# isi-vista/VistaOCR

Measured on AMD Instinct MI355X. Metric: line-images/sec (train, batch 32, 30x600 grey), higher is better.
Workload: dtype f32 (the LSTM's large GEMMs as bf16x6 products: fp32 operands split exactly into three bf16 planes, six bf16 MFMAs per fp32 product, fp32 accumulate; VOCR_LSTM_GEMM=f32 restores the f32-MFMA kernels); 1 GPU; configs[1]: 32 synthetic 1x30x600 grey lines per GPU, 20 labels/line, V=96, 3xBiLSTM-512, train() = H2D of the batch + fwd+CTC+bwd+allreduce+clamp+Adam, loss returned as a float; widths=600 .. 600 px, mean 600, conv_dtype=fp32, global_batch=32, parallelism=dp1, ranks_seen=1, backend=none, per_rank_rng=seed 1234 + 1000*rank after an identical init

## Files before the change

### include/vocr.h

```cpp
#ifndef VOCR_H
#define VOCR_H
#include <stddef.h>
#include <stdint.h>

#ifdef __cplusplus
extern "C" {
#endif

#define VOCR_OK          0
#define VOCR_EINVAL     -1
#define VOCR_ELAUNCH    -2
#define VOCR_ENODEVICE  -3
#define VOCR_ECOMM      -4


const char* vocr_last_error(void);
#define VOCR_ABI_VERSION 5
int  vocr_abi_version(void);
int  vocr_profile_range_push(const char* name);
int  vocr_profile_range_pop(void);
int  vocr_device_count(void);

int vocr_conv3x3_pack_weights(const float* w, float* wpack_fwd, float* wpack_dgrad, int cout, int cin, void* stream);
int vocr_conv3x3_fwd(const float* x, const float* wpack, const float* bias, float* y,
// ... 111 lines not shown

size_t vocr_gemm_x6_planes_bytes(int rows, int k);
int vocr_gemm_x6_split(const float* x, const float* x2, int seg, int seg_axis, const float* mask, long ld, int rows, int k, int k_contiguous,
                       void* planes, void* stream);
size_t vocr_gemm_x6_workspace_bytes(int m, int n, int k);
#define VOCR_GEMM_X6_PLAN_INTS 9
int vocr_gemm_x6_plan(int m, int n, int k, int b_rows, int b_row0, int b_row0_2, int has_workspace, int* plan);
int vocr_gemm_x6(const void* a_planes, int a_rows, int a_k, int a_row0, int a_kk0, const void* b_planes, int b_rows, int b_k, int b_row0, int b_kk0,
                 int m, int n, int k, float* c0, float* c1, int csplit, int rsplit, int ldc, const float* bias0, const float* bias1, int relu,
                 void* workspace, void* stream);

int vocr_gemm_x6_two_views(const void* a_planes, int a_rows, int a_k, int a_row0, const void* b_planes, int b_rows, int b_k, int m, int n, int k,
                           int rsplit, int a_kk0, int b_row0, int b_kk0, int a_kk0_2, int b_row0_2, int b_kk0_2, float* c0, float* c1, int ldc,
                           void* workspace, void* stream);

size_t vocr_gemm_h3_planes_bytes(int rows, int k);
int vocr_gemm_h3_split(const float* x, const float* x2, int seg, int seg_axis, const float* mask, long ld, int rows, int k, int k_contiguous,
                       float bound, void* planes, void* stream);
int vocr_gemm_h3(const void* a_planes, int a_rows, int a_k, int a_row0, int a_kk0, const void* b_planes, int b_rows, int b_k, int b_row0, int b_kk0,
                 int m, int n, int k, float* c0, float* c1, int csplit, int rsplit, int ldc, const float* bias0, const float* bias1, int relu,
                 void* workspace, void* stream);
int vocr_gemm_h3_two_views(const void* a_planes, int a_rows, int a_k, int a_row0, const void* b_planes, int b_rows, int b_k, int m, int n, int k,
                           int rsplit, int a_kk0, int b_row0, int b_kk0, int a_kk0_2, int b_row0_2, int b_kk0_2, float* c0, float* c1, int ldc,
                           void* workspace, void* stream);

int vocr_lstm_packed_supported(int b, int h);
int vocr_seq_rowmap(const int32_t* lens, int t, int b, int rows, int32_t* to_packed, int32_t* to_dense, void* stream);
int vocr_gather_rows(const float* src, float* dst, const int32_t* map, long nrows, int n, const float* fill, void* stream);
size_t vocr_gather_rows_fill_grad_workspace_bytes(int n);
int vocr_gather_rows_fill_grad(const float* dout, const int32_t* map, long nrows, int n, float* dfill, void* workspace, void* stream);
// ... 119 lines not shown
```

### vistaocr_amd/_lib.py

```python
import ctypes
import os
from ctypes import c_char_p, c_float, c_int, c_size_t, c_uint32, c_uint64, c_void_p

_HERE = os.path.dirname(os.path.abspath(__file__))
LIB_PATH = os.path.join(_HERE, "csrc", "libvocr.so")

P, I, F, Z, U64, U32 = c_void_p, c_int, c_float, c_size_t, c_uint64, c_uint32

SIGNATURES = {
    "vocr_last_error": (c_char_p, []),
    "vocr_abi_version": (I, []),
    "vocr_device_count": (I, []),
    "vocr_profile_range_push": (I, [c_char_p]),
    "vocr_profile_range_pop": (I, []),
    "vocr_conv3x3_pack_weights": (I, [P, P, P, I, I, P]),
    "vocr_conv3x3_fwd": (I, [P, P, P, P, I, I, I, I, I, P]),
    "vocr_conv3x3_wgrad_workspace_bytes": (Z, [I, I, I, I, I]),
    "vocr_conv3x3_wgrad": (I, [P, P, P, P, I, I, I, I, I, P]),
    "vocr_conv3x3_wino_supported": (I, [I, I]),
    "vocr_conv3x3_wino_pack_floats": (Z, [I, I]),
    "vocr_conv3x3_wino_pack_weights": (I, [P, P, P, I, I, P]),
    "vocr_conv3x3_wino_fwd": (I, [P, P, P, P, I, I, I, I, I, P]),
    "vocr_conv3x3_wino_plan": (I, [I, I, I, I, I]),
    "vocr_conv3x3_wgrad_wino_workspace_bytes": (Z, [I, I, I, I, I]),
# ... 28 lines not shown
    "vocr_bn_relu_fracpool2x2_fwd": (I, [P, P, P, P, P, P, P, P, I, I, I, I, I, I, P]),
    "vocr_fracpool2x2_bwd": (I, [P, P, P, I, I, I, I, I, I, P]),
    "vocr_relu_maxpool2_fwd": (I, [P, P, P, I, I, I, I, P]),
    "vocr_relu_maxpool2_bwd": (I, [P, P, P, P, I, I, I, I, P]),
    "vocr_gemm_workspace_bytes": (Z, [I, I, I, I]),
    "vocr_gemm": (I, [I, I, I, I, I, P, I, P, I, P, I, P, I, I, P, Z, P]),
    "vocr_gemm_plan": (I, [I, I, I, I, I, I, I, I, I, I, I, Z, I, I, I, P]),
    "vocr_gemm_pair_workspace_bytes": (Z, [I, I, I, I]),
    "vocr_gemm_pair": (I, [I, I, I, I, I, I, P, P, I, P, P, I, P, P, I, P, P, I, P, Z, P]),
    "vocr_gemm_x6_planes_bytes": (Z, [I, I]),
    "vocr_gemm_x6_split": (I, [P, P, I, I, P, ctypes.c_long, I, I, I, P, P]),
    "vocr_gemm_x6_workspace_bytes": (Z, [I, I, I]),
    "vocr_gemm_x6_plan": (I, [I, I, I, I, I, I, I, P]),
    "vocr_gemm_x6": (I, [P, I, I, I, I, P, I, I, I, I, I, I, I, P, P, I, I, I, P, P, I, P, P]),
    "vocr_gemm_x6_two_views": (I, [P, I, I, I, P, I, I, I, I, I, I, I, I, I, I, I, I, P, P, I, P, P]),
    "vocr_gemm_h3_two_views": (I, [P, I, I, I, P, I, I, I, I, I, I, I, I, I, I, I, I, P, P, I, P, P]),
    "vocr_gemm_h3_planes_bytes": (Z, [I, I]),
    "vocr_gemm_h3_split": (I, [P, P, I, I, P, ctypes.c_long, I, I, I, ctypes.c_float, P, P]),
    "vocr_gemm_h3": (I, [P, I, I, I, I, P, I, I, I, I, I, I, I, P, P, I, I, I, P, P, I, P, P]),
    "vocr_colsum_workspace_bytes": (Z, [I, I]),
    "vocr_colsum": (I, [P, P, I, I, P, P]),
    "vocr_relu_bwd": (I, [P, P, P, Z, P]),
    "vocr_bchw_to_wbch": (I, [P, P, I, I, I, I, P]),
    "vocr_wbch_to_bchw": (I, [P, P, I, I, I, I, P]),
    "vocr_mul": (I, [P, P, P, Z, P]),
    "vocr_add": (I, [P, P, P, Z, P]),
    "vocr_scale_dev": (I, [P, P, P, Z, P]),
    "vocr_dropout_fwd": (I, [P, P, P, Z, F, U64, P]),
    "vocr_dropout_mask": (I, [P, Z, F, U64, P]),
    "vocr_lstm_workspace_bytes": (Z, [I, I, I]),
# ... 138 lines not shown
```

### vistaocr_amd/csrc/gemm_x6.hip

```cpp
#include "vocr_common.h"

namespace {

typedef __bf16 bf16x8 __attribute__((ext_vector_type(8)));
typedef unsigned u32x4x __attribute__((ext_vector_type(4)));
#define X6_LDS_PTR(p) ((__attribute__((address_space(3))) void*)(p))
#define X6_H(v) __builtin_bit_cast(f16x8, v)

constexpr int X6_BM = 256;
constexpr int X6_LDS = 144 * 1024;

__device__ __forceinline__ void split3(float a, __bf16& b0, __bf16& b1, __bf16& b2) {
    b0 = (__bf16)a;
    if (__builtin_isinf((float)b0) && !__builtin_isinf(a)) b0 = __builtin_bit_cast(__bf16, (unsigned short)(__float_as_uint(a) >> 16));
    const float r1 = a - (float)b0;
    b1 = (__bf16)r1;
    const float r2 = r1 - (float)b1;
    b2 = (__bf16)r2;
}

struct X6Src {
    const float* x;
    const float* x2;
    const float* mask;
// ... 187 lines not shown
    const float* sb;
};

constexpr int X6_PANEL = 4;
__device__ __forceinline__ void x6_tile_of(int t, int mtiles, int ntiles, int& mt, int& nt) {
    const int panel = t / (X6_PANEL * ntiles), within = t - panel * X6_PANEL * ntiles;
    const int rows = min(X6_PANEL, mtiles - panel * X6_PANEL);
    nt = within / rows;
    mt = panel * X6_PANEL + within - nt * rows;
}
__device__ __forceinline__ int x6_xcd_chunked(int i, int n) {
    const int xcd = i & 7, j = i >> 3, c = n >> 3, rr = n & 7;
    return xcd * c + min(xcd, rr) + j;
}

template <int NCT, int NP>
__global__ __launch_bounds__(512) void gemm_x6_kernel(const X6Args g) {
    constexpr int BN = 32 * NCT;
    constexpr int TM = NCT == 4 ? 2 : 4, TN = 2;
    constexpr int NA = 8 * NP;
    constexpr int NFRAG = NA + NP * NCT;
    constexpr int NS = NP == 3 ? (NCT == 4 ? 4 : 3) : (NCT == 4 ? 6 : 4);
    constexpr int STAGE = NFRAG * 1024;
    constexpr int NDMA_MAX = (NFRAG + 7) / 8;
    constexpr int NDMA_LO = NFRAG / 8, NDMA_ODD = NFRAG % 8;
    extern __shared__ __attribute__((aligned(1024))) unsigned char lds[];
    const int tid = threadIdx.x, lane = tid & 63;
    const int wave = __builtin_amdgcn_readfirstlane(tid >> 6);
    const int wm = NCT == 4 ? (wave & 3) : (wave & 1), wn = NCT == 4 ? (wave >> 2) : (wave >> 1);
    const int v = x6_xcd_chunked(blockIdx.x, gridDim.x);
    const int ltile = v % g.ntile_launch, split = v / g.ntile_launch;
    int mt, nt;
    x6_tile_of(g.tile0 + ltile, g.mtiles, g.ntiles, mt, nt);
    const int s_beg = split * g.stages_per_split, s_end = min(g.nkk, s_beg + g.stages_per_split);
    if (s_beg >= s_end) return;

    const long pa = (long)g.RTa * g.KKa * 1024, pb = (long)g.RTb * g.KKb * 1024;
    const bool alt = mt >= g.alt_mt;
    const int a_kk0 = alt ? g.a_kk0_alt : g.a_kk0, b_kk0 = alt ? g.b_kk0_alt : g.b_kk0, b_rt0 = alt ? g.b_rt0_alt : g.b_rt0;
    const __amdgpu_buffer_rsrc_t ra = __builtin_amdgcn_make_buffer_rsrc((void*)g.a, 0, (int)(NP * pa), 0x00020000);
    const __amdgpu_buffer_rsrc_t rb = __builtin_amdgcn_make_buffer_rsrc((void*)g.b, 0, (int)(NP * pb), 0x00020000);
    const int voff = lane * 16;
    auto dma_one = [&](int s, int slot, int i) {
        const int f = wave + 8 * i;
        unsigned char* dst = lds + slot * STAGE + f * 1024;
        const bool live = s < s_end;
#if defined(X6_CUT) && (X6_CUT & 16)
        s = s_beg;
#endif
        if (f < NA) {
            const long off = (f >> 3) * pa + ((long)(g.a_rt0 + 8 * mt + (f & 7)) * g.KKa + a_kk0 + s) * 1024;
            __builtin_amdgcn_raw_ptr_buffer_load_lds(ra, X6_LDS_PTR(dst), 16, live ? voff : -16, live ? (int)off : 0, 0, 0);
        } else {
            const int fb = f - NA;
            const long off = (fb / NCT) * pb + ((long)(b_rt0 + NCT * nt + (fb % NCT)) * g.KKb + b_kk0 + s) * 1024;
            __builtin_amdgcn_raw_ptr_buffer_load_lds(rb, X6_LDS_PTR(dst), 16, live ? voff : -16, live ? (int)off : 0, 0, 0);
        }
    };
    auto dma_nth = [&](int s, int slot, int i) {
        if (8 * i + 7 < NFRAG || wave + 8 * i < NFRAG) dma_one(s, slot, i);
    };

    f32x16 acc[TM][TN];
#pragma unroll
    for (int i = 0; i < TM; ++i)
#pragma unroll
        for (int j = 0; j < TN; ++j)
#pragma unroll
            for (int r = 0; r < 16; ++r) acc[i][j][r] = 0.f;

#pragma unroll
    for (int i = 0; i < NS - 1; ++i)
#pragma unroll
        for (int d = 0; d < NDMA_MAX; ++d) dma_nth(s_beg + i, i, d);
#ifndef X6_CUT
#define X6_CUT 0
#endif
    int slot = 0;
    for (int s = s_beg; s < s_end; ++s) {
        if (!(X6_CUT & 1) && !(X6_CUT & 32)) {
            static_assert((NS - 2) * (NDMA_LO + (NDMA_ODD ? 1 : 0)) < 16, "vmcnt immediate");
            if (NDMA_ODD && wave < NDMA_ODD) __builtin_amdgcn_s_waitcnt(0x0F70 | ((NS - 2) * (NDMA_LO + 1)));
            else __builtin_amdgcn_s_waitcnt(0x0F70 | ((NS - 2) * NDMA_LO));
        }
        if (!(X6_CUT & 8)) __builtin_amdgcn_s_barrier();
        const unsigned char* base = lds + slot * STAGE + lane * 16;
        bf16x8 af[TM][NP], bf[TN][NP];
#pragma unroll
        for (int tn = 0; tn < TN; ++tn)
#pragma unroll
            for (int p = 0; p < NP; ++p) bf[tn][p] = *(const bf16x8*)(base + (NA + p * NCT + TN * wn + tn) * 1024);
#pragma unroll
        for (int tm = 0; tm < TM; ++tm)
#pragma unroll
            for (int p = 0; p < NP; ++p) af[tm][p] = *(const bf16x8*)(base + (p * 8 + TM * wm + tm) * 1024);
        __builtin_amdgcn_sched_barrier(0);
        const int snext = s + NS - 1, slot_next = slot == 0 ? NS - 1 : slot - 1;
        int d = 0;
#pragma unroll
        for (int tm = 0; tm < TM; ++tm)
#pragma unroll
            for (int tn = 0; tn < TN; ++tn) {
                if (!(X6_CUT & 2)) {
                    if constexpr (NP == 3) {
                        acc[tm][tn] = __builtin_amdgcn_mfma_f32_32x32x16_bf16(af[tm][1], bf[tn][1], acc[tm][tn], 0, 0, 0);
                        acc[tm][tn] = __builtin_amdgcn_mfma_f32_32x32x16_bf16(af[tm][0], bf[tn][2], acc[tm][tn], 0, 0, 0);
                        acc[tm][tn] = __builtin_amdgcn_mfma_f32_32x32x16_bf16(af[tm][2], bf[tn][0], acc[tm][tn], 0, 0, 0);
                    } else {
                        acc[tm][tn] = __builtin_amdgcn_mfma_f32_32x32x16_f16(X6_H(af[tm][0]), X6_H(bf[tn][1]), acc[tm][tn], 0, 0, 0);
                        acc[tm][tn] = __builtin_amdgcn_mfma_f32_32x32x16_f16(X6_H(af[tm][1]), X6_H(bf[tn][0]), acc[tm][tn], 0, 0, 0);
// ... 173 lines not shown
struct X6Route { X6Plan p; bool wide_ok; int ncu, main_tiles, cut_tiles, ksplit, stages_per_split; size_t ws_bytes; };
X6Route x6_route(int m, int n, int nkk, int RTb, int b_rt0, int b_rt0_alt, bool can_cut) {
    X6Route r;
    r.ncu = x6_cu_count();
    const X6Plan p4 = x6_plan(4, m, n, nkk, r.ncu, can_cut), p8 = x6_plan(8, m, n, nkk, r.ncu, can_cut);
    r.wide_ok = b_rt0 + 8 * p8.ntiles <= RTb && b_rt0_alt + 8 * p8.ntiles <= RTb;
    r.p = (r.wide_ok && p8.cost < p4.cost) ? p8 : p4;
    r.main_tiles = r.p.ks > 1 ? r.p.full : r.p.tiles;
    r.cut_tiles = r.p.ks > 1 ? r.p.rem : 0;
    r.stages_per_split = r.p.ks > 1 ? vocr_cdiv(nkk, r.p.ks) : nkk;
    r.ksplit = vocr_cdiv(nkk, r.stages_per_split);
    r.ws_bytes = r.p.ks > 1 ? (size_t)r.ksplit * r.cut_tiles * X6_BM * (32 * r.p.nct) * sizeof(float) : 0;
    return r;
}

template <int NCT, int NP>
void x6_launch(X6Args g, const X6Route& r, void* workspace, hipStream_t s) {
    g.ntiles = r.p.ntiles;
    if (r.main_tiles > 0) {
        g.tile0 = 0; g.ntile_launch = r.main_tiles; g.ksplit = 1; g.stages_per_split = g.nkk; g.slab = nullptr;
        gemm_x6_kernel<NCT, NP><<<r.main_tiles, 512, X6_LDS, s>>>(g);
    }
    if (r.cut_tiles > 0) {
        g.tile0 = r.main_tiles; g.ntile_launch = r.cut_tiles;
        g.stages_per_split = r.stages_per_split;
        g.ksplit = r.ksplit;
        g.slab = (float*)workspace;
        gemm_x6_kernel<NCT, NP><<<r.cut_tiles * r.ksplit, 512, X6_LDS, s>>>(g);
        gemm_x6_reduce_kernel<NCT><<<r.cut_tiles * (NCT == 4 ? 32 : 64), 256, 0, s>>>(g);
    }
}
}

struct X6AltViews { int a_kk0, b_row0, b_kk0; };
template <int NP>
static int x6_gemm_impl(const char* name, const void* a_planes, int a_rows, int a_k, int a_row0, int a_kk0, const void* b_planes, int b_rows, int b_k,
                        int b_row0, int b_kk0, int m, int n, int k, float* c0, float* c1, int csplit, int rsplit, int ldc, const float* bias0,
                        const float* bias1, int relu, void* workspace, void* stream, const X6AltViews* alt = nullptr) {
    VOCR_CHECK_ARG(a_planes && b_planes && c0, "%s: null pointer", name);
    VOCR_CHECK_ARG(m > 0 && n > 0 && k > 0 && ldc > 0 && k % 16 == 0, "%s: bad shape (k %% 16 == 0)", name);
    VOCR_CHECK_ARG(a_row0 % 32 == 0 && b_row0 % 32 == 0 && a_row0 >= 0 && b_row0 >= 0 && a_kk0 >= 0 && b_kk0 >= 0, "%s: views start on tile boundaries", name);
    VOCR_CHECK_ARG((csplit <= 0 && rsplit <= 0) || c1, "%s: a second output needs c1", name);
    VOCR_CHECK_ARG(!(csplit > 0 && rsplit > 0), "%s: one cut, along the columns or along the rows", name);
    X6Args g;
    g.a = a_planes; g.b = b_planes;
    g.c[0] = c0; g.c[1] = c1 ? c1 : c0;
    g.bias[0] = bias0; g.bias[1] = bias1;
    g.M = m; g.N = n; g.nkk = k / 16;
    g.RTa = x6_rt(a_rows); g.KKa = x6_kk(a_k); g.RTb = x6_rt(b_rows); g.KKb = x6_kk(b_k);
    g.a_rt0 = a_row0 / 32; g.a_kk0 = a_kk0; g.b_rt0 = b_row0 / 32; g.b_kk0 = b_kk0;
    g.alt_mt = 1 << 30; g.a_kk0_alt = a_kk0; g.b_rt0_alt = g.b_rt0; g.b_kk0_alt = b_kk0;
    if (alt) {
        VOCR_CHECK_ARG(rsplit > 0 && rsplit % X6_BM == 0 && alt->b_row0 % 32 == 0 && alt->b_row0 >= 0 && alt->a_kk0 >= 0 && alt->b_kk0 >= 0,
                       "%s: a second view set needs a row cut on a 256-row tile boundary and views on tile boundaries", name);
        g.alt_mt = rsplit / X6_BM; g.a_kk0_alt = alt->a_kk0; g.b_rt0_alt = alt->b_row0 / 32; g.b_kk0_alt = alt->b_kk0;
    }
    g.mtiles = vocr_cdiv(m, X6_BM);
    g.csplit = csplit > 0 ? csplit : (1 << 30);
    g.rsplit = rsplit > 0 ? rsplit : (1 << 30);
    g.ldc = ldc;
    g.relu = relu;
    g.sa = NP == 2 ? (const float*)((const unsigned char*)a_planes + (size_t)NP * g.RTa * g.KKa * 1024) : nullptr;
    g.sb = NP == 2 ? (const float*)((const unsigned char*)b_planes + (size_t)NP * g.RTb * g.KKb * 1024) : nullptr;
    const X6Route route = x6_route(m, n, g.nkk, g.RTb, g.b_rt0, g.b_rt0_alt, workspace != nullptr);
    const X6Plan& p = route.p;
    VOCR_CHECK_ARG(g.a_rt0 + 8 * g.mtiles <= g.RTa && g.b_rt0 + p.nct * p.ntiles <= g.RTb && g.a_kk0 + g.nkk <= g.KKa && g.b_kk0 + g.nkk <= g.KKb,
                   "%s: the view leaves its plane set", name);
    VOCR_CHECK_ARG(g.b_rt0_alt + p.nct * p.ntiles <= g.RTb && g.a_kk0_alt + g.nkk <= g.KKa && g.b_kk0_alt + g.nkk <= g.KKb,
                   "%s: the second view leaves its plane set", name);
    static VocrPerDevice lds_set;
    const void* const big[] = {(const void*)gemm_x6_kernel<4, NP>, (const void*)gemm_x6_kernel<8, NP>};
    if (vocr_allow_dynamic_lds(big, 2, X6_LDS, &lds_set, name) != VOCR_OK) return VOCR_ELAUNCH;
    if (p.nct == 8) x6_launch<8, NP>(g, route, workspace, (hipStream_t)stream);
    else x6_launch<4, NP>(g, route, workspace, (hipStream_t)stream);
    VOCR_CHECK_LAUNCH(name);
    return VOCR_OK;
}

extern "C" int vocr_gemm_x6_plan(int m, int n, int k, int b_rows, int b_row0, int b_row0_2, int has_workspace, int* plan) {
    VOCR_CHECK_ARG(plan != nullptr, "vocr_gemm_x6_plan: null pointer");
    VOCR_CHECK_ARG(m > 0 && n > 0 && k > 0 && k % 16 == 0 && b_rows > 0, "vocr_gemm_x6_plan: bad shape (k %% 16 == 0)");
    VOCR_CHECK_ARG(b_row0 >= 0 && b_row0 % 32 == 0 && (b_row0_2 < 0 || b_row0_2 % 32 == 0), "vocr_gemm_x6_plan: views start on tile boundaries");
    const X6Route r = x6_route(m, n, k / 16, x6_rt(b_rows), b_row0 / 32, (b_row0_2 < 0 ? b_row0 : b_row0_2) / 32, has_workspace != 0);
    plan[0] = r.p.nct;
    plan[1] = r.p.tiles;
    plan[2] = r.main_tiles;
    plan[3] = r.cut_tiles;
    plan[4] = r.ksplit;
    plan[5] = r.stages_per_split;
// ... 11 lines not shown
}
extern "C" int vocr_gemm_h3(const void* a_planes, int a_rows, int a_k, int a_row0, int a_kk0, const void* b_planes, int b_rows, int b_k, int b_row0,
                            int b_kk0, int m, int n, int k, float* c0, float* c1, int csplit, int rsplit, int ldc, const float* bias0,
                            const float* bias1, int relu, void* workspace, void* stream) {
    return x6_gemm_impl<2>("vocr_gemm_h3", a_planes, a_rows, a_k, a_row0, a_kk0, b_planes, b_rows, b_k, b_row0, b_kk0, m, n, k, c0, c1, csplit, rsplit, ldc,
                           bias0, bias1, relu, workspace, stream);
}

extern "C" int vocr_gemm_x6_two_views(const void* a_planes, int a_rows, int a_k, int a_row0, const void* b_planes, int b_rows, int b_k, int m, int n, int k,
                                      int rsplit, int a_kk0, int b_row0, int b_kk0, int a_kk0_2, int b_row0_2, int b_kk0_2, float* c0, float* c1, int ldc,
                                      void* workspace, void* stream) {
    const X6AltViews alt = {a_kk0_2, b_row0_2, b_kk0_2};
    return x6_gemm_impl<3>("vocr_gemm_x6_two_views", a_planes, a_rows, a_k, a_row0, a_kk0, b_planes, b_rows, b_k, b_row0, b_kk0, m, n, k, c0, c1, 0, rsplit, ldc,
                           nullptr, nullptr, 0, workspace, stream, &alt);
}
extern "C" int vocr_gemm_h3_two_views(const void* a_planes, int a_rows, int a_k, int a_row0, const void* b_planes, int b_rows, int b_k, int m, int n, int k,
                                      int rsplit, int a_kk0, int b_row0, int b_kk0, int a_kk0_2, int b_row0_2, int b_kk0_2, float* c0, float* c1, int ldc,
                                      void* workspace, void* stream) {
    const X6AltViews alt = {a_kk0_2, b_row0_2, b_kk0_2};
    return x6_gemm_impl<2>("vocr_gemm_h3_two_views", a_planes, a_rows, a_k, a_row0, a_kk0, b_planes, b_rows, b_k, b_row0, b_kk0, m, n, k, c0, c1, 0, rsplit, ldc,
                           nullptr, nullptr, 0, workspace, stream, &alt);
}
```

### vistaocr_amd/ops.py

```python
import math

import torch

from . import _lib
from ._lib import call, prof_range


def _stream():
    return torch.cuda.current_stream().cuda_stream


def _ranged(name):
    def deco(fn):
        if not _lib.ROCTX:
            return fn

        def wrapped(*a, **k):
            with prof_range(name):
                return fn(*a, **k)
        wrapped.__name__ = fn.__name__
        wrapped.__doc__ = fn.__doc__
        return wrapped
    return deco

# ... 568 lines not shown
         int(workspace_bytes), int(nprob), int(nseg), int(bool(tiles_only)), out)
    v = list(out)
    return dict(kernel=GEMM_PLAN_KERNELS[v[0]], vec=bool(v[1]), n_whole=v[2], pieces_per_tile=v[3], k_per_piece=v[4], panels=v[5],
                groups=v[6], ksplit=v[7], k_per_split=v[8], max_row_tiles=v[9], launches=v[10], workspace_bytes=v[11])


def gemm_pair(mode, ta, tb, m, n, k, a0, a1, lda, b0, b1, ldb, c0, c1, ldc, bias0=None, bias1=None, relu=False):
    nb = _lib.load().vocr_gemm_pair_workspace_bytes(m, n, k, int(mode))
    ws = _ws(nb, c0.device) if nb else None
    call("vocr_gemm_pair", int(mode), int(ta), int(tb), m, n, k, _p(a0), _p(a1), lda, _p(b0), _p(b1), ldb, _p(c0), _p(c1), ldc,
         _p(bias0), _p(bias1), int(relu), _p(ws), nb, _stream())


_GEMM_X6 = _exp("VOCR_GEMM_X6", "1") == "1"
_X6_TWO_VIEWS = _exp("VOCR_X6_TWO_VIEWS", "1") == "1"
LSTM_GEMM_MODES = ("bf16x6", "fp16x3", "f32")
_LSTM_GEMM = _os.environ.get("VOCR_LSTM_GEMM", "bf16x6")
if _LSTM_GEMM not in LSTM_GEMM_MODES:
    raise ValueError("VOCR_LSTM_GEMM=%r: one of %s" % (_LSTM_GEMM, ", ".join(LSTM_GEMM_MODES)))
_X6_ENTRY = {"bf16x6": ("vocr_gemm_x6_planes_bytes", "vocr_gemm_x6_split", "vocr_gemm_x6", "vocr_gemm_x6_two_views"),
             "fp16x3": ("vocr_gemm_h3_planes_bytes", "vocr_gemm_h3_split", "vocr_gemm_h3", "vocr_gemm_h3_two_views")}


def set_lstm_gemm(mode):
    global _LSTM_GEMM
    if mode not in LSTM_GEMM_MODES:
        raise ValueError("lstm gemm mode %r: one of %s" % (mode, ", ".join(LSTM_GEMM_MODES)))
    prev, _LSTM_GEMM = _LSTM_GEMM, mode
    return prev

# ... 8 lines not shown

def x6_planes(x, rows, k, k_contiguous, ld, x2=None, seg=0, axis=0, mask=None, scheme=None, bound=0.0):
    scheme = scheme or lstm_gemm()
    nbytes, split = _X6_ENTRY[scheme][:2]
    lib = _lib.load()
    buf = torch.empty(getattr(lib, nbytes)(int(rows), int(k)) // 2, dtype=torch.int16, device=x.device)
    if scheme == "fp16x3":
        call(split, _p(x), _p(x2), int(seg), int(axis), _p(mask), int(ld), int(rows), int(k), int(bool(k_contiguous)), float(bound), _p(buf), _stream())
    else:
        call(split, _p(x), _p(x2), int(seg), int(axis), _p(mask), int(ld), int(rows), int(k), int(bool(k_contiguous)), _p(buf), _stream())
    buf.x6_scheme = scheme
    return buf


def gemm_x6(a, a_rows, a_k, b, b_rows, b_k, m, n, k, c0, ldc, c1=None, csplit=0, rsplit=0, bias0=None, bias1=None, a_row0=0, a_kk0=0, b_row0=0,
            b_kk0=0, relu=False):
    scheme = getattr(a, "x6_scheme", None)
    if scheme is None or scheme != getattr(b, "x6_scheme", None):
        raise RuntimeError("gemm_x6: operands from different splits (%r, %r)" % (scheme, getattr(b, "x6_scheme", None)))
    ws = _ws(_lib.load().vocr_gemm_x6_workspace_bytes(m, n, k), c0.device)
    call(_X6_ENTRY[scheme][2], _p(a), int(a_rows), int(a_k), int(a_row0), int(a_kk0), _p(b), int(b_rows), int(b_k), int(b_row0), int(b_kk0), int(m), int(n),
         int(k), _p(c0), _p(c1), int(csplit), int(rsplit), int(ldc), _p(bias0), _p(bias1), int(relu), _p(ws), _stream())


def gemm_x6_plan(m, n, k, b_rows=None, b_row0=0, b_row0_2=-1, workspace=True):
    out = (_ctypes.c_int * 9)()
    call("vocr_gemm_x6_plan", int(m), int(n), int(k), int(n if b_rows is None else b_rows), int(b_row0), int(b_row0_2), int(bool(workspace)), out)
    v = list(out)
    return dict(tile=v[0], tiles=v[1], whole_tiles=v[2], cut_tiles=v[3], ksplit=v[4], stages_per_split=v[5], wide_ok=bool(v[6]), cus=v[7],
                workspace_bytes=v[8])


def gemm_x6_two_views(a, a_rows, a_k, b, b_rows, b_k, m, n, k, rsplit, views0, views1, c0, c1, ldc, a_row0=0):
    scheme = getattr(a, "x6_scheme", None)
    if scheme is None or scheme != getattr(b, "x6_scheme", None):
        raise RuntimeError("gemm_x6_two_views: operands from different splits (%r, %r)" % (scheme, getattr(b, "x6_scheme", None)))
    ws = _ws(_lib.load().vocr_gemm_x6_workspace_bytes(m, n, k), c0.device)
    call(_X6_ENTRY[scheme][3], _p(a), int(a_rows), int(a_k), int(a_row0), _p(b), int(b_rows), int(b_k), int(m), int(n), int(k), int(rsplit),
         int(views0[0]), int(views0[1]), int(views0[2]), int(views1[0]), int(views1[1]), int(views1[2]), _p(c0), _p(c1), int(ldc), _p(ws), _stream())


def colsum(x2d, out=None):
    m, n = x2d.shape
    out = out if out is not None else torch.empty(n, dtype=torch.float32, device=x2d.device)
    nb = _lib.load().vocr_colsum_workspace_bytes(m, n)
    ws = _ws(nb, x2d.device) if nb else None
    call("vocr_colsum", _p(x2d), _p(out), m, n, _p(ws), _stream())
    return out


def transpose2d(x):
    r, c = x.shape
# ... 188 lines not shown
            bsum, wt_f, wt_r = prep.lstm[w_hh_f.data_ptr()]
            if wt_f is not None:
                ctx.wt = (wt_f, wt_r)
        else:
            bsum = torch.empty(2, 4 * H, dtype=torch.float32, device=dev)
            call("vocr_add", _p(b_ih_f), _p(b_hh_f), _p(bsum[0]), 4 * H, _stream())
            call("vocr_add", _p(b_ih_r), _p(b_hh_r), _p(bsum[1]), 4 * H, _stream())
        y = (torch.zeros if rows else torch.empty)(R, 2 * H, dtype=torch.float32, device=dev)
        gates = torch.empty(2, R, 4 * H, dtype=torch.float32, device=dev)
        cell = torch.empty(2, R, H, dtype=torch.float32, device=dev)
        ws = _ws(lib.vocr_lstm_workspace_bytes(T, B, H), dev)
        G = 4 * H

        ctx.x6 = x6_layer_ok(T, B, H, rows)
        ctx.x6_wt = None
        if pre is None and ctx.x6 and din >= 512:
            if prep is not None and w_ih_f.data_ptr() in prep.x6w:
                wk, ctx.x6_wt = prep.x6w[w_ih_f.data_ptr()]
            else:
                wk, ctx.x6_wt = x6_weight_planes(w_ih_f, w_ih_r, torch.is_grad_enabled())
            xa = x6_planes(x, R, din, True, din, bound=x_bound)
            gemm_x6(xa, R, din, wk, 2 * G, din, R, 2 * G, din, xproj[0], G, c1=xproj[1], csplit=G, bias0=bsum[0], bias1=bsum[1])
        elif pre is None:
            gemm_pair(0, 0, 1, R, G, din, x, x, din, w_ih_f, w_ih_r, din, xproj[0], xproj[1], G, bias0=bsum[0], bias1=bsum[1])
        mask = drop_mask
        if follow is not None:
            nf, nr = follow["w_ih"]
            wpack = follow.get("wpack")
            if wpack is None:
                wpack = lstm_xproj_pack(nf, nr)
            nbias = follow.get("bias")
            if mask is None and drop_p and float(drop_p) > 0.0:
                mask = torch.empty_like(y)
                call("vocr_dropout_mask", _p(mask), mask.numel(), float(drop_p), int(drop_seed), _stream())
            planes = torch.empty(2, 2, R, G, dtype=torch.float32, device=dev)
            p0, p1 = (pre if pre is not None else (xproj, None))
            call("vocr_lstm_fwd_lead", _p(p0), _p(p1), _p(w_hh_f), _p(w_hh_r), _p(lens_dev), _p(y), _p(gates), _p(cell), _p(ws), T, B, H, R if rows else 0,
# ... 45 lines not shown
        if rows:
            call("vocr_lstm_bwd_packed", _p(dy), _p(mask), _p(wt_f), _p(wt_r), _p(lens_dev), _p(gates), _p(cell), _p(dg), _p(dbias), _p(ws),
                 T, B, H, R, _p(health(dev)), _stream())
        elif parts:
            call("vocr_lstm_bwd_parts", _p(dy), _p(mask), _p(wt_f), _p(wt_r), _p(lens_dev), _p(gates), _p(cell), _p(dg), _p(ws),
                 T, B, H, _p(health(dev)), _stream())
        else:
            if mask is not None:
                dym = torch.empty_like(dy)
                call("vocr_mul", _p(dy), _p(mask), _p(dym), dy.numel(), _stream())
                dy = dym
            call("vocr_lstm_bwd_bias", _p(dy), _p(wt_f), _p(wt_r), _p(lens_dev), _p(gates), _p(cell), _p(dg), _p(dbias), _p(ws),
                 T, B, H, _p(health(dev)), _stream())
        G = 4 * H
        dx = None
        if ctx.needs_input_grad[0]:
            dx = torch.empty_like(x)
            if ctx.x6 and din >= 512:
                wt = ctx.x6_wt if ctx.x6_wt is not None else x6_weight_planes(w_ih_f, w_ih_r, True)[1]
                da = x6_planes(dg[0], R, 2 * G, True, G, x2=dg[1], seg=G, axis=0)
                gemm_x6(da, R, 2 * G, wt, din, 2 * G, R, din, 2 * G, dx, din)
            else:
                gemm_pair(1, 0, 0, R, din, G, dg[0], dg[1], G, w_ih_f, w_ih_r, din, dx, None, din)

        params = (w_ih_f, w_hh_f, ctx.b_refs[0], ctx.b_refs[1], w_ih_r, w_hh_r, ctx.b_refs[2], ctx.b_refs[3])
        sinks = _sinks(params) if ctx.direct_grads else None
        direct = sinks is not None

        def weight_grads(outs, co=0):
            dwi_f, dwh_f, dbi_f, dbh_f, dwi_r, dwh_r, dbi_r, dbh_r = outs
            if parts:
                call("vocr_lstm_bias_from_parts", _p(dbias), _p(ws), T, B, H, _stream())
            sh = 4 if rows else B
            if ctx.x6:
                k16 = (R + 15) // 16 * 16
                dgt = x6_planes(dg[0], 2 * G, R, False, G, x2=dg[1], seg=G, axis=1)
                xt = x6_planes(x, din, R, False, din, bound=ctx.x_bound)
                gemm_x6(dgt, 2 * G, R, xt, din, R, 2 * G, din, k16, dwi_f, din, c1=dwi_r, rsplit=G)
                if T > 1 and sh % 16 == 0 and (R - sh) % 16 == 0 and G % 256 == 0:
                    yt = x6_planes(y, 2 * H, R, False, 2 * H, bound=1.0)
                    if _X6_TWO_VIEWS:
                        gemm_x6_two_views(dgt, 2 * G, R, yt, 2 * H, R, 2 * G, H, R - sh, G, (sh // 16, 0, 0), (0, H, sh // 16), dwh_f, dwh_r, H)
                    else:
                        gemm_x6(dgt, 2 * G, R, yt, 2 * H, R, G, H, R - sh, dwh_f, H, a_row0=0, a_kk0=sh // 16, b_row0=0, b_kk0=0)
                        gemm_x6(dgt, 2 * G, R, yt, 2 * H, R, G, H, R - sh, dwh_r, H, a_row0=G, a_kk0=0, b_row0=H, b_kk0=sh // 16)
                elif T > 1:
                    gemm_pair(co, 1, 0, G, H, R - sh, dg[0][sh:], dg[1], G, y, y[sh:, H:], 2 * H, dwh_f, dwh_r, H)
                else:
# ... 7 lines not shown
            gemm_pair(co, 1, 0, G, din, R, dg[0], dg[1], G, x, x, din, dwi_f, dwi_r, din)
            if T > 1:
                m = R - sh
                gemm_pair(co, 1, 0, G, H, m, dg[0][sh:], dg[1], G, y, y[sh:, H:], 2 * H, dwh_f, dwh_r, H)
            else:
                dwh_f.zero_()
                dwh_r.zero_()
            dbi_f.copy_(dbias[0])
            dbi_r.copy_(dbias[1])
            dbh_f.copy_(dbias[0])
            dbh_r.copy_(dbias[1])

        if direct and _SIDE_ENABLED and _exp("VOCR_LSTM_DW_OVERLAP", "1") == "1":
            side = side_stream()
            side.wait_stream(torch.cuda.current_stream())
            for t_ in (dg, x, y, dbias, ws):
                t_.record_stream(side)
            with torch.cuda.stream(side):
                weight_grads(sinks)
            mark_side_pending()
            return (dx, None, None, None) + (None,) * 17
        if direct:
            weight_grads(sinks)
            return (dx, None, None, None) + (None,) * 17
        outs = [torch.empty_like(p) for p in params]
        weight_grads(outs)
        return (dx, None, None, None) + tuple(outs) + (None,) * 9


class CtcFn(torch.autograd.Function):

    @staticmethod
# ... 497 lines not shown
```

Baseline: 2313 line-images/sec.

## Reuse row-major bf16x6 planes for LSTM weight grads via transposing LDS reads

Adds a transposing mode to the bf16x6 GEMM kernel. It loads row-major plane tiles with swizzled DMA offsets and reads fragments with ds_read_tr16 so they come out transposed. The LSTM weight-gradient GEMMs now reuse the forward input planes (kept on ctx) and the dgrad dgate planes instead of re-splitting dgates, x and y into K-contiguous transposed plane sets. This removes several split kernels and their memory traffic per layer. In exchange it keeps the input planes alive from forward to backward, which costs memory, and the transposed LDS read path may be slower than the plain vector reads.

```diff
diff --git a/include/vocr.h b/include/vocr.h
--- a/include/vocr.h
+++ b/include/vocr.h
@@ -149,6 +149,13 @@
                            int rsplit, int a_kk0, int b_row0, int b_kk0, int a_kk0_2, int b_row0_2, int b_kk0_2, float* c0, float* c1, int ldc,
                            void* workspace, void* stream);
 
+int vocr_gemm_x6_t(const void* a_planes, int a_rows, int a_k, int a_row0, int a_kk0, int a_t, const void* b_planes, int b_rows, int b_k, int b_row0,
+                   int b_kk0, int b_t, int m, int n, int k, float* c0, float* c1, int csplit, int rsplit, int ldc, const float* bias0,
+                   const float* bias1, int relu, void* workspace, void* stream);
+int vocr_gemm_x6_two_views_t(const void* a_planes, int a_rows, int a_k, int a_row0, int a_t, const void* b_planes, int b_rows, int b_k, int b_t,
+                             int m, int n, int k, int rsplit, int a_kk0, int b_row0, int b_kk0, int a_kk0_2, int b_row0_2, int b_kk0_2, float* c0,
+                             float* c1, int ldc, void* workspace, void* stream);
+
 size_t vocr_gemm_h3_planes_bytes(int rows, int k);
 int vocr_gemm_h3_split(const float* x, const float* x2, int seg, int seg_axis, const float* mask, long ld, int rows, int k, int k_contiguous,
                        float bound, void* planes, void* stream);
diff --git a/vistaocr_amd/_lib.py b/vistaocr_amd/_lib.py
--- a/vistaocr_amd/_lib.py
+++ b/vistaocr_amd/_lib.py
@@ -66,6 +66,8 @@
     "vocr_gemm_x6_plan": (I, [I, I, I, I, I, I, I, P]),
     "vocr_gemm_x6": (I, [P, I, I, I, I, P, I, I, I, I, I, I, I, P, P, I, I, I, P, P, I, P, P]),
     "vocr_gemm_x6_two_views": (I, [P, I, I, I, P, I, I, I, I, I, I, I, I, I, I, I, I, P, P, I, P, P]),
+    "vocr_gemm_x6_t": (I, [P, I, I, I, I, I, P, I, I, I, I, I, I, I, I, P, P, I, I, I, P, P, I, P, P]),
+    "vocr_gemm_x6_two_views_t": (I, [P, I, I, I, I, P, I, I, I, I, I, I, I, I, I, I, I, I, I, P, P, I, P, P]),
     "vocr_gemm_h3_two_views": (I, [P, I, I, I, P, I, I, I, I, I, I, I, I, I, I, I, I, P, P, I, P, P]),
     "vocr_gemm_h3_planes_bytes": (Z, [I, I]),
     "vocr_gemm_h3_split": (I, [P, P, I, I, P, ctypes.c_long, I, I, I, ctypes.c_float, P, P]),
diff --git a/vistaocr_amd/csrc/gemm_x6.hip b/vistaocr_amd/csrc/gemm_x6.hip
--- a/vistaocr_amd/csrc/gemm_x6.hip
+++ b/vistaocr_amd/csrc/gemm_x6.hip
@@ -4,6 +4,8 @@
 
 typedef __bf16 bf16x8 __attribute__((ext_vector_type(8)));
 typedef unsigned u32x4x __attribute__((ext_vector_type(4)));
+typedef __bf16 bf16x4 __attribute__((ext_vector_type(4)));
+typedef short x6s16x4 __attribute__((ext_vector_type(4)));
 #define X6_LDS_PTR(p) ((__attribute__((address_space(3))) void*)(p))
 #define X6_H(v) __builtin_bit_cast(f16x8, v)
 
@@ -225,8 +227,9 @@
     return xcd * c + min(xcd, rr) + j;
 }
 
-template <int NCT, int NP>
+template <int NCT, int NP, bool TA = false, bool TB = false>
 __global__ __launch_bounds__(512) void gemm_x6_kernel(const X6Args g) {
+    static_assert(NP == 3 || (!TA && !TB), "fp16x3 carries one scale per plane-set row: no transposing mode");
     constexpr int BN = 32 * NCT;
     constexpr int TM = NCT == 4 ? 2 : 4, TN = 2;
     constexpr int NA = 8 * NP;
@@ -252,6 +255,7 @@
     const __amdgpu_buffer_rsrc_t ra = __builtin_amdgcn_make_buffer_rsrc((void*)g.a, 0, (int)(NP * pa), 0x00020000);
     const __amdgpu_buffer_rsrc_t rb = __builtin_amdgcn_make_buffer_rsrc((void*)g.b, 0, (int)(NP * pb), 0x00020000);
     const int voff = lane * 16;
+    const int voff_t = 512 * (lane >> 4) + 16 * (4 * (((lane >> 2) & 3) ^ (lane >> 4)) + (lane & 3));
     auto dma_one = [&](int s, int slot, int i) {
         const int f = wave + 8 * i;
         unsigned char* dst = lds + slot * STAGE + f * 1024;
@@ -260,12 +264,26 @@
         s = s_beg;
 #endif
         if (f < NA) {
-            const long off = (f >> 3) * pa + ((long)(g.a_rt0 + 8 * mt + (f & 7)) * g.KKa + a_kk0 + s) * 1024;
-            __builtin_amdgcn_raw_ptr_buffer_load_lds(ra, X6_LDS_PTR(dst), 16, live ? voff : -16, live ? (int)off : 0, 0, 0);
+            if constexpr (TA) {
+                const int ft = g.a_rt0 + 8 * mt + (f & 7), sa = a_kk0 + s;
+                const long off = (f >> 3) * pa + ((long)(sa >> 1) * g.KKa + 2 * ft) * 1024 + (sa & 1) * 256;
+                const bool lv = live && 2 * ft < g.KKa;
+                __builtin_amdgcn_raw_ptr_buffer_load_lds(ra, X6_LDS_PTR(dst), 16, lv ? voff_t : -16, lv ? (int)off : 0, 0, 0);
+            } else {
+                const long off = (f >> 3) * pa + ((long)(g.a_rt0 + 8 * mt + (f & 7)) * g.KKa + a_kk0 + s) * 1024;
+                __builtin_amdgcn_raw_ptr_buffer_load_lds(ra, X6_LDS_PTR(dst), 16, live ? voff : -16, live ? (int)off : 0, 0, 0);
+            }
         } else {
             const int fb = f - NA;
-            const long off = (fb / NCT) * pb + ((long)(b_rt0 + NCT * nt + (fb % NCT)) * g.KKb + b_kk0 + s) * 1024;
-            __builtin_amdgcn_raw_ptr_buffer_load_lds(rb, X6_LDS_PTR(dst), 16, live ? voff : -16, live ? (int)off : 0, 0, 0);
+            if constexpr (TB) {
+                const int ft = b_rt0 + NCT * nt + (fb % NCT), sb = b_kk0 + s;
+                const long off = (fb / NCT) * pb + ((long)(sb >> 1) * g.KKb + 2 * ft) * 1024 + (sb & 1) * 256;
+                const bool lv = live && 2 * ft < g.KKb;
+                __builtin_amdgcn_raw_ptr_buffer_load_lds(rb, X6_LDS_PTR(dst), 16, lv ? voff_t : -16, lv ? (int)off : 0, 0, 0);
+            } else {
+                const long off = (fb / NCT) * pb + ((long)(b_rt0 + NCT * nt + (fb % NCT)) * g.KKb + b_kk0 + s) * 1024;
+                __builtin_amdgcn_raw_ptr_buffer_load_lds(rb, X6_LDS_PTR(dst), 16, live ? voff : -16, live ? (int)off : 0, 0, 0);
+            }
         }
     };
     auto dma_nth = [&](int s, int slot, int i) {
@@ -296,15 +314,29 @@
         }
         if (!(X6_CUT & 8)) __builtin_amdgcn_s_barrier();
         const unsigned char* base = lds + slot * STAGE + lane * 16;
+        const int tc = 2 * ((lane >> 4) & 1) + ((lane >> 1) & 1), tfg = 2 * (lane >> 5);
+        const unsigned char* base_t0 = lds + slot * STAGE + 256 * tc + 64 * (tfg ^ tc) + 16 * ((lane >> 2) & 3) + 8 * (lane & 1);
+        const unsigned char* base_t1 = lds + slot * STAGE + 256 * tc + 64 * ((tfg + 1) ^ tc) + 16 * ((lane >> 2) & 3) + 8 * (lane & 1);
+        auto frag_t = [&](int fr) {
+            const x6s16x4 lo = __builtin_amdgcn_ds_read_tr16_b64_v4i16((__attribute__((address_space(3))) x6s16x4*)(base_t0 + fr * 1024));
+            const x6s16x4 hi = __builtin_amdgcn_ds_read_tr16_b64_v4i16((__attribute__((address_space(3))) x6s16x4*)(base_t1 + fr * 1024));
+            return __builtin_shufflevector(__builtin_bit_cast(bf16x4, lo), __builtin_bit_cast(bf16x4, hi), 0, 1, 2, 3, 4, 5, 6, 7);
+        };
         bf16x8 af[TM][NP], bf[TN][NP];
 #pragma unroll
         for (int tn = 0; tn < TN; ++tn)
 #pragma unroll
-            for (int p = 0; p < NP; ++p) bf[tn][p] = *(const bf16x8*)(base + (NA + p * NCT + TN * wn + tn) * 1024);
+            for (int p = 0; p < NP; ++p) {
+                if constexpr (TB) bf[tn][p] = frag_t(NA + p * NCT + TN * wn + tn);
+                else bf[tn][p] = *(const bf16x8*)(base + (NA + p * NCT + TN * wn + tn) * 1024);
+            }
 #pragma unroll
         for (int tm = 0; tm < TM; ++tm)
 #pragma unroll
-            for (int p = 0; p < NP; ++p) af[tm][p] = *(const bf16x8*)(base + (p * 8 + TM * wm + tm) * 1024);
+            for (int p = 0; p < NP; ++p) {
+                if constexpr (TA) af[tm][p] = frag_t(p * 8 + TM * wm + tm);
+                else af[tm][p] = *(const bf16x8*)(base + (p * 8 + TM * wm + tm) * 1024);
+            }
         __builtin_amdgcn_sched_barrier(0);
         const int snext = s + NS - 1, slot_next = slot == 0 ? NS - 1 : slot - 1;
         int d = 0;
@@ -508,21 +540,30 @@
     return r;
 }
 
-template <int NCT, int NP>
+template <int NCT, int NP, bool TA = false, bool TB = false>
 void x6_launch(X6Args g, const X6Route& r, void* workspace, hipStream_t s) {
     g.ntiles = r.p.ntiles;
     if (r.main_tiles > 0) {
         g.tile0 = 0; g.ntile_launch = r.main_tiles; g.ksplit = 1; g.stages_per_split = g.nkk; g.slab = nullptr;
-        gemm_x6_kernel<NCT, NP><<<r.main_tiles, 512, X6_LDS, s>>>(g);
+        gemm_x6_kernel<NCT, NP, TA, TB><<<r.main_tiles, 512, X6_LDS, s>>>(g);
     }
     if (r.cut_tiles > 0) {
         g.tile0 = r.main_tiles; g.ntile_launch = r.cut_tiles;
         g.stages_per_split = r.stages_per_split;
         g.ksplit = r.ksplit;
         g.slab = (float*)workspace;
-        gemm_x6_kernel<NCT, NP><<<r.cut_tiles * r.ksplit, 512, X6_LDS, s>>>(g);
+        gemm_x6_kernel<NCT, NP, TA, TB><<<r.cut_tiles * r.ksplit, 512, X6_LDS, s>>>(g);
         gemm_x6_reduce_kernel<NCT><<<r.cut_tiles * (NCT == 4 ? 32 : 64), 256, 0, s>>>(g);
     }
+}
+template <int NP, bool TA, bool TB>
+int x6_launch_form(const X6Args& g, const X6Route& r, void* workspace, hipStream_t s, const char* name) {
+    static VocrPerDevice lds_set;
+    const void* const big[] = {(const void*)gemm_x6_kernel<4, NP, TA, TB>, (const void*)gemm_x6_kernel<8, NP, TA, TB>};
+    if (vocr_allow_dynamic_lds(big, 2, X6_LDS, &lds_set, name) != VOCR_OK) return VOCR_ELAUNCH;
+    if (r.p.nct == 8) x6_launch<8, NP, TA, TB>(g, r, workspace, s);
+    else x6_launch<4, NP, TA, TB>(g, r, workspace, s);
+    return VOCR_OK;
 }
 }
 
@@ -530,8 +571,9 @@
 template <int NP>
 static int x6_gemm_impl(const char* name, const void* a_planes, int a_rows, int a_k, int a_row0, int a_kk0, const void* b_planes, int b_rows, int b_k,
                         int b_row0, int b_kk0, int m, int n, int k, float* c0, float* c1, int csplit, int rsplit, int ldc, const float* bias0,
-                        const float* bias1, int relu, void* workspace, void* stream, const X6AltViews* alt = nullptr) {
+                        const float* bias1, int relu, void* workspace, void* stream, const X6AltViews* alt = nullptr, int a_t = 0, int b_t = 0) {
     VOCR_CHECK_ARG(a_planes && b_planes && c0, "%s: null pointer", name);
+    VOCR_CHECK_ARG(NP == 3 || (!a_t && !b_t), "%s: the transposing mode is bf16x6 only", name);
     VOCR_CHECK_ARG(m > 0 && n > 0 && k > 0 && ldc > 0 && k % 16 == 0, "%s: bad shape (k %% 16 == 0)", name);
     VOCR_CHECK_ARG(a_row0 % 32 == 0 && b_row0 % 32 == 0 && a_row0 >= 0 && b_row0 >= 0 && a_kk0 >= 0 && b_kk0 >= 0, "%s: views start on tile boundaries", name);
     VOCR_CHECK_ARG((csplit <= 0 && rsplit <= 0) || c1, "%s: a second output needs c1", name);
@@ -541,7 +583,8 @@
     g.c[0] = c0; g.c[1] = c1 ? c1 : c0;
     g.bias[0] = bias0; g.bias[1] = bias1;
     g.M = m; g.N = n; g.nkk = k / 16;
-    g.RTa = x6_rt(a_rows); g.KKa = x6_kk(a_k); g.RTb = x6_rt(b_rows); g.KKb = x6_kk(b_k);
+    g.RTa = a_t ? x6_rt(a_k) : x6_rt(a_rows); g.KKa = a_t ? x6_kk(a_rows) : x6_kk(a_k);
+    g.RTb = b_t ? x6_rt(b_k) : x6_rt(b_rows); g.KKb = b_t ? x6_kk(b_rows) : x6_kk(b_k);
     g.a_rt0 = a_row0 / 32; g.a_kk0 = a_kk0; g.b_rt0 = b_row0 / 32; g.b_kk0 = b_kk0;
     g.alt_mt = 1 << 30; g.a_kk0_alt = a_kk0; g.b_rt0_alt = g.b_rt0; g.b_kk0_alt = b_kk0;
     if (alt) {
@@ -556,17 +599,27 @@
     g.relu = relu;
     g.sa = NP == 2 ? (const float*)((const unsigned char*)a_planes + (size_t)NP * g.RTa * g.KKa * 1024) : nullptr;
     g.sb = NP == 2 ? (const float*)((const unsigned char*)b_planes + (size_t)NP * g.RTb * g.KKb * 1024) : nullptr;
-    const X6Route route = x6_route(m, n, g.nkk, g.RTb, g.b_rt0, g.b_rt0_alt, workspace != nullptr);
+    const X6Route route = x6_route(m, n, g.nkk, x6_rt(b_rows), g.b_rt0, g.b_rt0_alt, workspace != nullptr);
     const X6Plan& p = route.p;
-    VOCR_CHECK_ARG(g.a_rt0 + 8 * g.mtiles <= g.RTa && g.b_rt0 + p.nct * p.ntiles <= g.RTb && g.a_kk0 + g.nkk <= g.KKa && g.b_kk0 + g.nkk <= g.KKb,
-                   "%s: the view leaves its plane set", name);
-    VOCR_CHECK_ARG(g.b_rt0_alt + p.nct * p.ntiles <= g.RTb && g.a_kk0_alt + g.nkk <= g.KKa && g.b_kk0_alt + g.nkk <= g.KKb,
-                   "%s: the second view leaves its plane set", name);
-    static VocrPerDevice lds_set;
-    const void* const big[] = {(const void*)gemm_x6_kernel<4, NP>, (const void*)gemm_x6_kernel<8, NP>};
-    if (vocr_allow_dynamic_lds(big, 2, X6_LDS, &lds_set, name) != VOCR_OK) return VOCR_ELAUNCH;
-    if (p.nct == 8) x6_launch<8, NP>(g, route, workspace, (hipStream_t)stream);
-    else x6_launch<4, NP>(g, route, workspace, (hipStream_t)stream);
+    const bool a_ok = a_t ? (g.a_kk0 + g.nkk <= 2 * g.RTa && 2l * g.a_rt0 + vocr_cdiv(m, 16) <= g.KKa)
+                          : (g.a_rt0 + 8 * g.mtiles <= g.RTa && g.a_kk0 + g.nkk <= g.KKa);
+    const bool a_alt_ok = g.a_kk0_alt + g.nkk <= (a_t ? 2 * g.RTa : g.KKa);
+    const bool b_ok = b_t ? (g.b_kk0 + g.nkk <= 2 * g.RTb && 2l * g.b_rt0 + vocr_cdiv(n, 16) <= g.KKb)
+                          : (g.b_rt0 + p.nct * p.ntiles <= g.RTb && g.b_kk0 + g.nkk <= g.KKb);
+    const bool b_alt_ok = b_t ? (g.b_kk0_alt + g.nkk <= 2 * g.RTb && 2l * g.b_rt0_alt + vocr_cdiv(n, 16) <= g.KKb)
+                              : (g.b_rt0_alt + p.nct * p.ntiles <= g.RTb && g.b_kk0_alt + g.nkk <= g.KKb);
+    VOCR_CHECK_ARG(a_ok && b_ok, "%s: the view leaves its plane set", name);
+    VOCR_CHECK_ARG(a_alt_ok && b_alt_ok, "%s: the second view leaves its plane set", name);
+    int rc = VOCR_OK;
+    if constexpr (NP == 3) {
+        if (a_t && b_t) rc = x6_launch_form<3, true, true>(g, route, workspace, (hipStream_t)stream, name);
+        else if (a_t) rc = x6_launch_form<3, true, false>(g, route, workspace, (hipStream_t)stream, name);
+        else if (b_t) rc = x6_launch_form<3, false, true>(g, route, workspace, (hipStream_t)stream, name);
+        else rc = x6_launch_form<3, false, false>(g, route, workspace, (hipStream_t)stream, name);
+    } else {
+        rc = x6_launch_form<NP, false, false>(g, route, workspace, (hipStream_t)stream, name);
+    }
+    if (rc != VOCR_OK) return rc;
     VOCR_CHECK_LAUNCH(name);
     return VOCR_OK;
 }
@@ -608,6 +661,20 @@
     return x6_gemm_impl<3>("vocr_gemm_x6_two_views", a_planes, a_rows, a_k, a_row0, a_kk0, b_planes, b_rows, b_k, b_row0, b_kk0, m, n, k, c0, c1, 0, rsplit, ldc,
                            nullptr, nullptr, 0, workspace, stream, &alt);
 }
+
+extern "C" int vocr_gemm_x6_t(const void* a_planes, int a_rows, int a_k, int a_row0, int a_kk0, int a_t, const void* b_planes, int b_rows, int b_k,
+                              int b_row0, int b_kk0, int b_t, int m, int n, int k, float* c0, float* c1, int csplit, int rsplit, int ldc,
+                              const float* bias0, const float* bias1, int relu, void* workspace, void* stream) {
+    return x6_gemm_impl<3>("vocr_gemm_x6_t", a_planes, a_rows, a_k, a_row0, a_kk0, b_planes, b_rows, b_k, b_row0, b_kk0, m, n, k, c0, c1, csplit, rsplit, ldc,
+                           bias0, bias1, relu, workspace, stream, nullptr, a_t, b_t);
+}
+extern "C" int vocr_gemm_x6_two_views_t(const void* a_planes, int a_rows, int a_k, int a_row0, int a_t, const void* b_planes, int b_rows, int b_k, int b_t,
+                                        int m, int n, int k, int rsplit, int a_kk0, int b_row0, int b_kk0, int a_kk0_2, int b_row0_2, int b_kk0_2, float* c0,
+                                        float* c1, int ldc, void* workspace, void* stream) {
+    const X6AltViews alt = {a_kk0_2, b_row0_2, b_kk0_2};
+    return x6_gemm_impl<3>("vocr_gemm_x6_two_views_t", a_planes, a_rows, a_k, a_row0, a_kk0, b_planes, b_rows, b_k, b_row0, b_kk0, m, n, k, c0, c1, 0, rsplit,
+                           ldc, nullptr, nullptr, 0, workspace, stream, &alt, a_t, b_t);
+}
 extern "C" int vocr_gemm_h3_two_views(const void* a_planes, int a_rows, int a_k, int a_row0, const void* b_planes, int b_rows, int b_k, int m, int n, int k,
                                       int rsplit, int a_kk0, int b_row0, int b_kk0, int a_kk0_2, int b_row0_2, int b_kk0_2, float* c0, float* c1, int ldc,
                                       void* workspace, void* stream) {
diff --git a/vistaocr_amd/ops.py b/vistaocr_amd/ops.py
--- a/vistaocr_amd/ops.py
+++ b/vistaocr_amd/ops.py
@@ -606,6 +606,7 @@
 
 _GEMM_X6 = _exp("VOCR_GEMM_X6", "1") == "1"
 _X6_TWO_VIEWS = _exp("VOCR_X6_TWO_VIEWS", "1") == "1"
+_X6_TR = _exp("VOCR_X6_TR", "1") == "1"
 LSTM_GEMM_MODES = ("bf16x6", "fp16x3", "f32")
 _LSTM_GEMM = _os.environ.get("VOCR_LSTM_GEMM", "bf16x6")
 if _LSTM_GEMM not in LSTM_GEMM_MODES:
@@ -644,11 +645,17 @@
 
 
 def gemm_x6(a, a_rows, a_k, b, b_rows, b_k, m, n, k, c0, ldc, c1=None, csplit=0, rsplit=0, bias0=None, bias1=None, a_row0=0, a_kk0=0, b_row0=0,
-            b_kk0=0, relu=False):
+            b_kk0=0, relu=False, a_t=False, b_t=False):
     scheme = getattr(a, "x6_scheme", None)
     if scheme is None or scheme != getattr(b, "x6_scheme", None):
         raise RuntimeError("gemm_x6: operands from different splits (%r, %r)" % (scheme, getattr(b, "x6_scheme", None)))
     ws = _ws(_lib.load().vocr_gemm_x6_workspace_bytes(m, n, k), c0.device)
+    if a_t or b_t:
+        if scheme != "bf16x6":
+            raise RuntimeError("gemm_x6: the transposing mode is bf16x6 only (%r)" % (scheme,))
+        call("vocr_gemm_x6_t", _p(a), int(a_rows), int(a_k), int(a_row0), int(a_kk0), int(bool(a_t)), _p(b), int(b_rows), int(b_k), int(b_row0), int(b_kk0),
+             int(bool(b_t)), int(m), int(n), int(k), _p(c0), _p(c1), int(csplit), int(rsplit), int(ldc), _p(bias0), _p(bias1), int(relu), _p(ws), _stream())
+        return
     call(_X6_ENTRY[scheme][2], _p(a), int(a_rows), int(a_k), int(a_row0), int(a_kk0), _p(b), int(b_rows), int(b_k), int(b_row0), int(b_kk0), int(m), int(n),
          int(k), _p(c0), _p(c1), int(csplit), int(rsplit), int(ldc), _p(bias0), _p(bias1), int(relu), _p(ws), _stream())
 
@@ -661,11 +668,18 @@
                 workspace_bytes=v[8])
 
 
-def gemm_x6_two_views(a, a_rows, a_k, b, b_rows, b_k, m, n, k, rsplit, views0, views1, c0, c1, ldc, a_row0=0):
+def gemm_x6_two_views(a, a_rows, a_k, b, b_rows, b_k, m, n, k, rsplit, views0, views1, c0, c1, ldc, a_row0=0, a_t=False, b_t=False):
     scheme = getattr(a, "x6_scheme", None)
     if scheme is None or scheme != getattr(b, "x6_scheme", None):
         raise RuntimeError("gemm_x6_two_views: operands from different splits (%r, %r)" % (scheme, getattr(b, "x6_scheme", None)))
     ws = _ws(_lib.load().vocr_gemm_x6_workspace_bytes(m, n, k), c0.device)
+    if a_t or b_t:
+        if scheme != "bf16x6":
+            raise RuntimeError("gemm_x6_two_views: the transposing mode is bf16x6 only (%r)" % (scheme,))
+        call("vocr_gemm_x6_two_views_t", _p(a), int(a_rows), int(a_k), int(a_row0), int(bool(a_t)), _p(b), int(b_rows), int(b_k), int(bool(b_t)), int(m), int(n),
+             int(k), int(rsplit), int(views0[0]), int(views0[1]), int(views0[2]), int(views1[0]), int(views1[1]), int(views1[2]), _p(c0), _p(c1), int(ldc),
+             _p(ws), _stream())
+        return
     call(_X6_ENTRY[scheme][3], _p(a), int(a_rows), int(a_k), int(a_row0), _p(b), int(b_rows), int(b_k), int(m), int(n), int(k), int(rsplit),
          int(views0[0]), int(views0[1]), int(views0[2]), int(views1[0]), int(views1[1]), int(views1[2]), _p(c0), _p(c1), int(ldc), _p(ws), _stream())
 
@@ -884,6 +898,7 @@
 
         ctx.x6 = x6_layer_ok(T, B, H, rows)
         ctx.x6_wt = None
+        ctx.xa = None
         if pre is None and ctx.x6 and din >= 512:
             if prep is not None and w_ih_f.data_ptr() in prep.x6w:
                 wk, ctx.x6_wt = prep.x6w[w_ih_f.data_ptr()]
@@ -891,6 +906,8 @@
                 wk, ctx.x6_wt = x6_weight_planes(w_ih_f, w_ih_r, torch.is_grad_enabled())
             xa = x6_planes(x, R, din, True, din, bound=x_bound)
             gemm_x6(xa, R, din, wk, 2 * G, din, R, 2 * G, din, xproj[0], G, c1=xproj[1], csplit=G, bias0=bsum[0], bias1=bsum[1])
+            if _X6_TR and xa.x6_scheme == "bf16x6" and any(ctx.needs_input_grad):
+                ctx.xa = xa
         elif pre is None:
             gemm_pair(0, 0, 1, R, G, din, x, x, din, w_ih_f, w_ih_r, din, xproj[0], xproj[1], G, bias0=bsum[0], bias1=bsum[1])
         mask = drop_mask
@@ -966,6 +983,7 @@
                  T, B, H, _p(health(dev)), _stream())
         G = 4 * H
         dx = None
+        da = None
         if ctx.needs_input_grad[0]:
             dx = torch.empty_like(x)
             if ctx.x6 and din >= 512:
@@ -984,6 +1002,29 @@
             if parts:
                 call("vocr_lstm_bias_from_parts", _p(dbias), _p(ws), T, B, H, _stream())
             sh = 4 if rows else B
+            if ctx.x6 and _X6_TR and lstm_gemm() == "bf16x6":
+                k16 = (R + 15) // 16 * 16
+                dar = da if da is not None else x6_planes(dg[0], R, 2 * G, True, G, x2=dg[1], seg=G, axis=0)
+                xar = ctx.xa if ctx.xa is not None else x6_planes(x, R, din, True, din)
+                gemm_x6(dar, 2 * G, R, xar, din, R, 2 * G, din, k16, dwi_f, din, c1=dwi_r, rsplit=G, a_t=True, b_t=True)
+                if T > 1 and sh % 16 == 0 and (R - sh) % 16 == 0 and G % 256 == 0:
+                    ya = x6_planes(y, R, 2 * H, True, 2 * H)
+                    if _X6_TWO_VIEWS:
+                        gemm_x6_two_views(dar, 2 * G, R, ya, 2 * H, R, 2 * G, H, R - sh, G, (sh // 16, 0, 0), (0, H, sh // 16), dwh_f, dwh_r, H,
+                                          a_t=True, b_t=True)
+                    else:
+                        gemm_x6(dar, 2 * G, R, ya, 2 * H, R, G, H, R - sh, dwh_f, H, a_row0=0, a_kk0=sh // 16, b_row0=0, b_kk0=0, a_t=True, b_t=True)
+                        gemm_x6(dar, 2 * G, R, ya, 2 * H, R, G, H, R - sh, dwh_r, H, a_row0=G, a_kk0=0, b_row0=H, b_kk0=sh // 16, a_t=True, b_t=True)
+                elif T > 1:
+                    gemm_pair(co, 1, 0, G, H, R - sh, dg[0][sh:], dg[1], G, y, y[sh:, H:], 2 * H, dwh_f, dwh_r, H)
+                else:
+                    dwh_f.zero_()
+                    dwh_r.zero_()
+                dbi_f.copy_(dbias[0])
+                dbi_r.copy_(dbias[1])
+                dbh_f.copy_(dbias[0])
+                dbh_r.copy_(dbias[1])
+                return
             if ctx.x6:
                 k16 = (R + 15) // 16 * 16
                 dgt = x6_planes(dg[0], 2 * G, R, False, G, x2=dg[1], seg=G, axis=1)
@@ -1021,8 +1062,9 @@
         if direct and _SIDE_ENABLED and _exp("VOCR_LSTM_DW_OVERLAP", "1") == "1":
             side = side_stream()
             side.wait_stream(torch.cuda.current_stream())
-            for t_ in (dg, x, y, dbias, ws):
-                t_.record_stream(side)
+            for t_ in (dg, x, y, dbias, ws, da, ctx.xa):
+                if t_ is not None:
+                    t_.record_stream(side)
             with torch.cuda.stream(side):
                 weight_grads(sinks)
             mark_side_pending()
```

Result: no change. 2318 line-images/sec, median of 6 (+0.2%).
